# amorim-cleison/sign-language-nlp

Hardware: AMD Instinct MI355X
Metric: train seq/s (batch=50,len=48) (higher is better)
Workload: dtype bf16x3; 1 GPU; cfg2: Transformer train step E512 H8 N6 F512 batch 50 len 48 |src| 3000 |tgt| 202 dropout 0.1, fwd+CE+bwd+clip(0.5)+SGD(m=.9); launch=eager stream launches (auto: timed both in 9 untimed pre-warmup steps + warmup), per_gpu=independent fit (grid shard)

## Files before the change

include/slnlp.h:

```cpp
#ifndef SLNLP_H
#define SLNLP_H

#include <stdint.h>

#ifdef __cplusplus
extern "C" {
#endif

#define SLNLP_OK 0
#define SLNLP_ERR_INVALID_ARG 1
#define SLNLP_ERR_LAUNCH 2
#define SLNLP_ERR_UNSUPPORTED 3

#define SLNLP_ABI_VERSION 1

const char* slnlp_last_error(void);
int slnlp_abi_version(void);

typedef struct slnlp_gemm_args {
    const float* A; int64_t lda; int32_t a_kmajor;
    const float* B; int64_t ldb; int32_t b_kmajor;
    float* C; int64_t ldc;
    int32_t M, N, K;
    const float* bias;
// ... 466 lines not shown
    float dropout;
    int32_t precision;
} slnlp_tf_config;

int slnlp_tf_num_params(const slnlp_tf_config* cfg);
int slnlp_tf_param_info(const slnlp_tf_config* cfg, int i, char* name, int64_t shape[2], int* ndim,
                        int64_t* offset);
int64_t slnlp_tf_arena_floats(const slnlp_tf_config* cfg);
int64_t slnlp_tf_workspace_bytes(const slnlp_tf_config* cfg);

typedef struct slnlp_tf_buffers {
    float* params;
    float* grads;
    float* momentum;
    const float* pe;
    void* workspace;
    unsigned long long* rng;
    float* lr;
    float* scalars;
} slnlp_tf_buffers;

typedef struct slnlp_tf_plan slnlp_tf_plan;
int slnlp_tf_create(const slnlp_tf_config* cfg, const slnlp_tf_buffers* buf, slnlp_tf_plan** out);
void slnlp_tf_destroy(slnlp_tf_plan* plan);
int slnlp_tf_forward(slnlp_tf_plan* plan, const int64_t* X, const int64_t* y, int B, int train,
                     float* logp, void* stream);
int slnlp_tf_seed_dlogp(slnlp_tf_plan* plan, const float* dlogp, void* stream);
int slnlp_tf_backward(slnlp_tf_plan* plan, void* stream);
int slnlp_tf_optim(slnlp_tf_plan* plan, float momentum, float max_norm, void* stream);
int slnlp_tf_optim_adam(slnlp_tf_plan* plan, float* exp_avg_sq, float beta1, float beta2, float eps, float weight_decay,
                        float max_norm, void* stream);
int slnlp_tf_train_step(slnlp_tf_plan* plan, const int64_t* X, const int64_t* y, int B,
                        float momentum, float max_norm, float* logp, void* stream);
int slnlp_tf_graph_capture_train(slnlp_tf_plan* plan, const int64_t* X, const int64_t* y, int B,
                                 float momentum, float max_norm, float* logp, void* stream);
int slnlp_tf_graph_launch(slnlp_tf_plan* plan, int B, void* stream);
int slnlp_tf_tap(slnlp_tf_plan* plan, const char* name, float* out, int64_t max_floats,
                 int64_t* n_out, void* stream);
int slnlp_tf_params_changed(slnlp_tf_plan* plan);
int slnlp_tf_debug_layout(const slnlp_tf_config* cfg, char* out, int64_t out_bytes);

int slnlp_tf_set_destroy_sync(slnlp_tf_plan* plan, int on);

#define SLNLP_UPDATE_SGD 0
#define SLNLP_UPDATE_ADAM 1
#define SLNLP_UPDATE_ADAMW 2
int slnlp_tf_set_criterion(slnlp_tf_plan* plan, const float* class_weight, float label_smoothing, int reduction, void* stream);
int slnlp_tf_set_update(slnlp_tf_plan* plan, int kind, float dampening, float weight_decay, int nesterov);
int slnlp_tf_set_param_groups(slnlp_tf_plan* plan, int n_segments, const int64_t* seg_begin, const int32_t* seg_group,
                              int n_groups, const float* weight_decay, const float* lr_dev, void* stream);
int slnlp_tf_set_averaging(slnlp_tf_plan* plan, float* avg, float* count, int kind, float decay);
int slnlp_tf_set_dmem_batched(slnlp_tf_plan* plan, int on);
int slnlp_tf_set_dec_ln_fused(slnlp_tf_plan* plan, int on);

int slnlp_set_thread_stream_policy(int serialise);
int slnlp_set_stream_policy(int serialise);

int slnlp_set_backward_passes(int wgrad, int dgrad);
int slnlp_get_backward_passes(int* wgrad, int* dgrad);

typedef struct slnlp_timed_launch { int32_t blocks, njobs, geometry; float us; } slnlp_timed_launch;
int slnlp_launch_timer_start(int max_records);
int slnlp_launch_timer_stop(slnlp_timed_launch* out, int max_out);

typedef struct slnlp_tf_lockstep slnlp_tf_lockstep;
int64_t slnlp_tf_lockstep_workspace_bytes(const slnlp_tf_config* cfg, int K);
int slnlp_tf_lockstep_create(slnlp_tf_plan** plans, int K, void* workspace, int64_t workspace_bytes, void* stream,
                             slnlp_tf_lockstep** out);
void slnlp_tf_lockstep_destroy(slnlp_tf_lockstep* group);
int slnlp_tf_lockstep_set_data(slnlp_tf_lockstep* group, int slot, const int64_t* const* X, const int64_t* const* y,
                               int64_t rows, float* const* logp, float* const* loss, void* stream);
int slnlp_tf_lockstep_step(slnlp_tf_lockstep* group, int slot, int64_t row0, int B, int step_index, int train,
                           float momentum, float max_norm, void* stream);
int slnlp_tf_lockstep_epoch(slnlp_tf_lockstep* group, int slot, int batch, int train, float momentum, float max_norm,
                            void* stream);
int slnlp_tf_lockstep_num_launches(slnlp_tf_lockstep* group, int slot, int B, int train);
int slnlp_tf_lockstep_set_adam(slnlp_tf_lockstep* group, float* const* exp_avg_sq, float beta1, float beta2, float eps,
                               float weight_decay);
int slnlp_tf_lockstep_set_lr_table(slnlp_tf_lockstep* group, const float* const* table, int n_steps, void* stream);
int slnlp_tf_lockstep_set_order(slnlp_tf_lockstep* group, int slot, const int64_t* const* order, int64_t n_visit, void* stream);
int slnlp_tf_lockstep_set_averaging(slnlp_tf_lockstep* group, float* const* avg, float* const* count, int kind, float decay);
int slnlp_tf_lockstep_set_destroy_sync(slnlp_tf_lockstep* group, int on);


typedef struct slnlp_rnn_config {
    int32_t lstm;
    int32_t E, Hd, N;
    int32_t Vs, Vt, B, S;
    int32_t pad_src, pad_tgt, bos_idx;
    float dropout;
    int32_t precision;
} slnlp_rnn_config;
int slnlp_rnn_num_params(const slnlp_rnn_config* cfg);
int slnlp_rnn_param_info(const slnlp_rnn_config* cfg, int i, char* name, int64_t shape[2], int* ndim, int64_t* offset);
int64_t slnlp_rnn_arena_floats(const slnlp_rnn_config* cfg);
int64_t slnlp_rnn_workspace_bytes(const slnlp_rnn_config* cfg);
typedef struct slnlp_rnn_plan slnlp_rnn_plan;
int slnlp_rnn_create(const slnlp_rnn_config* cfg, const slnlp_tf_buffers* buf, slnlp_rnn_plan** out);
void slnlp_rnn_destroy(slnlp_rnn_plan* plan);
int slnlp_rnn_forward(slnlp_rnn_plan* plan, const int64_t* X, const int64_t* y, const int64_t* lengths, int B,
                      int train, float* logp, void* stream);
int slnlp_rnn_set_persistent(slnlp_rnn_plan* plan, int on);
int slnlp_rnn_set_fused_backward(slnlp_rnn_plan* plan, int on);
int slnlp_rnn_health(slnlp_rnn_plan* plan, int* status);
int slnlp_rnn_seed_dlogp(slnlp_rnn_plan* plan, const float* dlogp, void* stream);
int slnlp_rnn_backward(slnlp_rnn_plan* plan, void* stream);
// ... 41 lines not shown
```

sign-language-nlp_amd/csrc/elementwise.hip:

```cpp
#include "common.hpp"
#include "launch.hpp"
#include "layernorm_row.hpp"

namespace slnlp {

__device__ __forceinline__ void embed_fwd_body(const long* __restrict__ ids, long ld_ids, int B, int S,
                                                        int E, int V, const float* __restrict__ table,
                                                        const float* __restrict__ pe, float* __restrict__ out,
                                                        float scale, float drop_p, unsigned drop_thr, int drop_site,
                                                        const unsigned long long* __restrict__ rng, long nan_idx,
                                                        PlaneOut po, unsigned char* __restrict__ keep_mask) {
    const int e4 = E >> 2;
    const long total = (long)B * S * e4;
    const float ik = 1.f / (1.f - drop_p);
    for (long idx = blockIdx.x * 256L + threadIdx.x; idx < total; idx += (long)gridDim.x * 256) {
        const int m = (int)(idx / e4), c = (int)(idx % e4) * 4;
        const int s = m / B, b = m % B;
        const long id = ids[(long)b * ld_ids + s];
        float4 v = make_float4(0.f, 0.f, 0.f, 0.f);
        if (id >= 0 && id < V) v = *reinterpret_cast<const float4*>(table + id * E + c);
        const float4 p = pe ? *reinterpret_cast<const float4*>(pe + (long)s * E + c) : make_float4(0.f, 0.f, 0.f, 0.f);
        v.x = v.x * scale + p.x; v.y = v.y * scale + p.y; v.z = v.z * scale + p.z; v.w = v.w * scale + p.w;
        if (drop_p > 0.f) {
            const bool k0 = dropout_keep(rng, drop_site, m, c + 0, drop_thr), k1 = dropout_keep(rng, drop_site, m, c + 1, drop_thr);
// ... 37 lines not shown
    const int M = B * S, lane = threadIdx.x & 63;
    const int m = blockIdx.x, m0 = (m / EMB_CHUNK) * EMB_CHUNK, t = m - m0, mine = m0 + lane;
    int my_id = -1;
    if (mine < M) {
        const long v = ids[(long)(mine % B) * ld_ids + (mine / B)];
        my_id = (v < 0 || v >= V) ? -1 : (int)v;
    }
    const float ik = 1.f / (1.f - drop_p);
    const int id = __builtin_amdgcn_readlane(my_id, __builtin_amdgcn_readfirstlane(t));
    const unsigned long long mask = __ballot(my_id == id && id >= 0);
    const bool first = id >= 0 && (mask & ((1ull << t) - 1ull)) == 0ull;
    if (threadIdx.x == 0) pid[m] = first ? id : -1;
    if (!first) return;
    __shared__ __attribute__((aligned(16))) float red[4][256];
    const int wave = threadIdx.x >> 6;
    const unsigned long long wmask = mask & (0xFFFFull << (16 * wave));
    for (int c0 = 0; c0 < E; c0 += 256) {
        const int c = c0 + lane * 4;
        float4 acc = make_float4(0.f, 0.f, 0.f, 0.f);
        if (c < E) {
            unsigned long long bits = wmask;
            while (bits) {
                int k[4];
#pragma unroll
                for (int u = 0; u < 4; ++u) {
                    k[u] = bits ? __ffsll((long long)bits) - 1 : -1;
                    bits &= bits - 1;
                }
                float4 g[4];
#pragma unroll
                for (int u = 0; u < 4; ++u)
                    g[u] = k[u] >= 0 ? load_dx_row(dx, m0 + k[u], E, c, drop_p, ik, drop_thr, drop_site, rng, keep_mask)
                                     : make_float4(0.f, 0.f, 0.f, 0.f);
#pragma unroll
                for (int u = 0; u < 4; ++u) { acc.x += g[u].x; acc.y += g[u].y; acc.z += g[u].z; acc.w += g[u].w; }
            }
        }
        if (c0 > 0) __syncthreads();
        *reinterpret_cast<float4*>(&red[wave][lane * 4]) = acc;
        __syncthreads();
        if (wave == 0 && c < E) {
            float4 r = *reinterpret_cast<const float4*>(&red[0][lane * 4]);
#pragma unroll
            for (int w = 1; w < 4; ++w) {
                const float4 q = *reinterpret_cast<const float4*>(&red[w][lane * 4]);
                r.x += q.x; r.y += q.y; r.z += q.z; r.w += q.w;
            }
            *reinterpret_cast<float4*>(partial + (long)m * E + c) = r;
        }
    }
}
SLNLP_ZKERNEL(embed_bwd_chunk_kernel, 256, embed_bwd_chunk_body)

__device__ __forceinline__ void embed_bwd_combine_body(const int* __restrict__ pid, int M, int E,
                                                                const float* __restrict__ partial,
                                                                float* __restrict__ dtable, float scale) {
    __shared__ int list[1024];
    __shared__ int nlist;
    const int m = blockIdx.x, tid = threadIdx.x;
    const int id = pid[m];
    if (id < 0) return;
    int dup = 0;
    for (int mm = tid; mm < m; mm += 256) dup |= (pid[mm] == id);
    if (__syncthreads_or(dup)) return;
    if (tid == 0) nlist = 0;
    __syncthreads();
    for (int base = m; base < M; base += 256) {
        const int mm = base + tid;
        const bool hit = mm < M && pid[mm] == id;
        const unsigned long long bal = __ballot(hit);
        __shared__ unsigned long long match[4];
        __syncthreads();
        if ((tid & 63) == 0) match[tid >> 6] = bal;
        __syncthreads();
        if (tid == 0) {
            int n = nlist;
            for (int w = 0; w < 4; ++w) {
                unsigned long long bits = match[w];
                while (bits && n < 1024) {
                    list[n++] = base + w * 64 + __ffsll((long long)bits) - 1;
                    bits &= bits - 1;
                }
            }
            nlist = n;
        }
        __syncthreads();
    }
    const int n = nlist;
    __shared__ __attribute__((aligned(16))) float red[4][256];
    const int wave = tid >> 6, lane = tid & 63, per = (n + 3) / 4;
    const int i0 = wave * per, i1 = (i0 + per < n) ? i0 + per : n;
    for (int c0 = 0; c0 < E; c0 += 256) {
        const int c = c0 + lane * 4;
        float4 acc = make_float4(0.f, 0.f, 0.f, 0.f);
        if (c < E) {
            for (int i = i0; i < i1; i += 4) {
                float4 g[4];
#pragma unroll
                for (int u = 0; u < 4; ++u)
                    g[u] = (i + u < i1) ? *reinterpret_cast<const float4*>(partial + (long)list[i + u] * E + c)
                                        : make_float4(0.f, 0.f, 0.f, 0.f);
#pragma unroll
                for (int u = 0; u < 4; ++u) { acc.x += g[u].x; acc.y += g[u].y; acc.z += g[u].z; acc.w += g[u].w; }
            }
        }
        if (c0 > 0) __syncthreads();
        *reinterpret_cast<float4*>(&red[wave][lane * 4]) = acc;
        __syncthreads();
        if (wave == 0 && c < E) {
            float4 r = *reinterpret_cast<const float4*>(&red[0][lane * 4]);
#pragma unroll
            for (int w = 1; w < 4; ++w) {
                const float4 q = *reinterpret_cast<const float4*>(&red[w][lane * 4]);
                r.x += q.x; r.y += q.y; r.z += q.z; r.w += q.w;
            }
            r.x *= scale; r.y *= scale; r.z *= scale; r.w *= scale;
            *reinterpret_cast<float4*>(dtable + (long)id * E + c) = r;
        }
    }
}
SLNLP_ZKERNEL(embed_bwd_combine_kernel, 256, embed_bwd_combine_body)

__device__ __forceinline__ void embed_bwd_small_body(const long* __restrict__ ids, long ld_ids, int B, int S, int E, int V,
                                                     const float* __restrict__ dx, float* __restrict__ dtable, float scale,
                                                     float drop_p, unsigned drop_thr, int drop_site,
                                                     const unsigned long long* __restrict__ rng) {
    const int M = B * S, lane = threadIdx.x & 63, m = blockIdx.x;
    int my_id = -1;
    if (lane < M) {
        const long v = ids[(long)(lane % B) * ld_ids + (lane / B)];
        my_id = (v < 0 || v >= V) ? -1 : (int)v;
    }
    if (m < V && __ballot(my_id == m) == 0ull) {
        for (int c = threadIdx.x * 4; c < E; c += 1024) *reinterpret_cast<float4*>(dtable + (long)m * E + c) = make_float4(0.f, 0.f, 0.f, 0.f);
    }
    if (m >= M) return;
    const float ik = 1.f / (1.f - drop_p);
    const int id = __builtin_amdgcn_readlane(my_id, __builtin_amdgcn_readfirstlane(m));
    const unsigned long long mask = __ballot(my_id == id && id >= 0);
    const bool first = id >= 0 && (mask & ((1ull << m) - 1ull)) == 0ull;
    if (!first) return;
    __shared__ __attribute__((aligned(16))) float red[4][256];
    const int wave = threadIdx.x >> 6;
    const unsigned long long wmask = mask & (0xFFFFull << (16 * wave));
    for (int c0 = 0; c0 < E; c0 += 256) {
        const int c = c0 + lane * 4;
        float4 acc = make_float4(0.f, 0.f, 0.f, 0.f);
        if (c < E) {
            unsigned long long bits = wmask;
            while (bits) {
                int k[4];
#pragma unroll
                for (int u = 0; u < 4; ++u) {
                    k[u] = bits ? __ffsll((long long)bits) - 1 : -1;
                    bits &= bits - 1;
                }
// ... 256 lines not shown
    LnPartialEntry e = table ? table[blockIdx.y] : single;
    const float* __restrict__ dy = as_global(e.dy);
    const float* __restrict__ x = as_global(e.x);
    const float* __restrict__ stats = as_global(e.stats);
    float* __restrict__ partial = as_global(e.partial);
    const int rows = e.dec ? rows_dec : rows_enc, chunk = e.dec ? chunk_dec : chunk_enc;
    const int c = threadIdx.x * 4;
    if (c >= E || (int)blockIdx.x >= (e.dec ? nchunk_dec : nchunk_enc)) return;
    const int r0 = blockIdx.x * chunk;
    const int r1 = r0 + chunk < rows ? r0 + chunk : rows;
    float4 ag = make_float4(0.f, 0.f, 0.f, 0.f), ab = make_float4(0.f, 0.f, 0.f, 0.f);
    auto add = [&](const float4& dd, const float4& vv, float mean, float rstd) {
        ag.x += dd.x * ((vv.x - mean) * rstd); ag.y += dd.y * ((vv.y - mean) * rstd);
        ag.z += dd.z * ((vv.z - mean) * rstd); ag.w += dd.w * ((vv.w - mean) * rstd);
        ab.x += dd.x; ab.y += dd.y; ab.z += dd.z; ab.w += dd.w;
    };
    int r = r0;
    for (; r + 8 <= r1; r += 8) {
        float4 dd[8], vv[8];
        float2 ms[8];
#pragma unroll
        for (int i = 0; i < 8; ++i) {
            dd[i] = *reinterpret_cast<const float4*>(dy + (long)(r + i) * E + c);
            vv[i] = *reinterpret_cast<const float4*>(x + (long)(r + i) * E + c);
            ms[i] = *reinterpret_cast<const float2*>(stats + 2 * (r + i));
        }
#pragma unroll
        for (int i = 0; i < 8; ++i) add(dd[i], vv[i], ms[i].x, ms[i].y);
    }
    for (; r < r1; ++r)
        add(*reinterpret_cast<const float4*>(dy + (long)r * E + c), *reinterpret_cast<const float4*>(x + (long)r * E + c), stats[2 * r], stats[2 * r + 1]);
    *reinterpret_cast<float4*>(partial + ((long)blockIdx.x * 2 + 0) * E + c) = ag;
    *reinterpret_cast<float4*>(partial + ((long)blockIdx.x * 2 + 1) * E + c) = ab;
}
SLNLP_ZKERNEL(ln_param_partial_kernel, 256, ln_param_partial_body)

__device__ __forceinline__ void ln_param_reduce_body(const slnlp_ln_reduce_entry* __restrict__ table) {
    __shared__ float red[2][4][64];
    const slnlp_ln_reduce_entry e = table[blockIdx.x];
    const int col = threadIdx.x & 63, grp = threadIdx.x >> 6, c = blockIdx.y * 64 + col;
    float g = 0.f, b = 0.f;
    if (c < e.E) {
        int k = grp;
        for (; k + 28 < e.nblk; k += 32) {
            float pg[8], pb[8];
#pragma unroll
            for (int u = 0; u < 8; ++u) {
                pg[u] = e.partial[((long)(k + 4 * u) * 2 + 0) * e.E + c];
                pb[u] = e.partial[((long)(k + 4 * u) * 2 + 1) * e.E + c];
            }
#pragma unroll
            for (int u = 0; u < 8; ++u) { g += pg[u]; b += pb[u]; }
        }
        for (; k < e.nblk; k += 4) {
            g += e.partial[((long)k * 2 + 0) * e.E + c];
            b += e.partial[((long)k * 2 + 1) * e.E + c];
        }
    }
    red[0][grp][col] = g;
    red[1][grp][col] = b;
    __syncthreads();
    if (grp == 0 && c < e.E) {
        e.dgamma[c] = (red[0][0][col] + red[0][1][col]) + (red[0][2][col] + red[0][3][col]);
        e.dbeta[c] = (red[1][0][col] + red[1][1][col]) + (red[1][2][col] + red[1][3][col]);
    }
}
SLNLP_ZKERNEL(ln_param_reduce_kernel, 256, ln_param_reduce_body)

int layernorm_fwd(const float* x, const float* gamma, const float* beta, int rows, int E, float eps, float* y,
                  float* stats, hipStream_t st, PlaneOut po) {
    SLNLP_CHECK_ARG(x && gamma && beta && y, "layernorm_fwd: null pointer");
    SLNLP_CHECK_ARG(rows > 0 && E > 0 && E % 4 == 0 && E <= LN_MAXU * 256, "layernorm_fwd: need E %% 4 == 0 and E <= %d, got rows=%d E=%d", LN_MAXU * 256, rows, E);
    SLNLP_TRY(zlaunch(layernorm_fwd_kernel, dim3(ceil_div(rows, 4)), 256, 0, st, "layernorm_fwd",
                      x, gamma, beta, rows, E, eps, y, stats, po));
    return 0;
}

static int ln_bwd_group(int rows) { return rows >= 1024 ? 4 : 1; }

bool ln_bwd_fused(int full_rows) { return ln_bwd_group(full_rows) == 4; }
int ln_partial_chunk(int rows) {
    int c = 16;
    while (ceil_div(rows, c) > SLNLP_LN_MAX_PARTIALS) c *= 2;
    return c;
}
int ln_bwd_blocks(int rows) { return ceil_div(rows, ln_partial_chunk(rows)); }

int ln_param_partial(const LnPartialEntry* table_dev, const LnPartialEntry* single_host, int n, int E, int rows_enc, int rows_dec, int full_rows_enc,
                     int full_rows_dec, hipStream_t st) {
    SLNLP_CHECK_ARG(n > 0 && E > 0 && E % 4 == 0 && E <= LN_MAXU * 256, "ln_param_partial: bad args");
    LnPartialEntry single;
    memset(&single, 0, sizeof(single));
    if (single_host) single = *single_host;
    const int ce = ln_partial_chunk(full_rows_enc > 0 ? full_rows_enc : 1), cd = ln_partial_chunk(full_rows_dec > 0 ? full_rows_dec : 1);
    const int ne = full_rows_enc > 0 && !(table_dev && ln_bwd_fused(full_rows_enc)) ? ceil_div(full_rows_enc, ce) : 0;
    const int nd = full_rows_dec > 0 ? ceil_div(full_rows_dec, cd) : 0;
    const int nb = std::max(ne, nd);
    if (nb == 0) return 0;
    const int threads = (ceil_div(E, 4) + 63) / 64 * 64;
    return zlaunch(ln_param_partial_kernel, dim3(nb, n), threads, 0, st, "ln_param_partial", table_dev, single, E,
                   rows_enc, rows_dec, ce, cd, ne, nd);
}

int layernorm_bwd(const float* dy, const float* x, const float* gamma, const float* stats, int rows, int E,
                  const float* add_to_dx, float* dx, float* dx_drop, float drop_p, int drop_site,
                  const unsigned long long* rng, float* partial, int* nblk_out, int full_rows, hipStream_t st,
                  PlaneOut po_dx, PlaneOut po_drop) {
    SLNLP_CHECK_ARG(dy && x && gamma && stats && dx, "layernorm_bwd: null pointer");
    SLNLP_CHECK_ARG(rows > 0 && E > 0 && E % 4 == 0 && E <= LN_MAXU * 256, "layernorm_bwd: need E %% 4 == 0 and E <= %d, got %d", LN_MAXU * 256, E);
// ... 362 lines not shown
```

sign-language-nlp_amd/csrc/tf_plan.hip:

```cpp
#include <map>
#include <string>
#include <vector>

#include "common.hpp"
#include "launch.hpp"
#include "tf_plan.hpp"

using namespace slnlp;

extern "C" {

int slnlp_tf_num_params(const slnlp_tf_config* cfg) {
    if (check_cfg(cfg)) return -1;
    return (int)build_layout(*cfg).ents.size();
}

int slnlp_tf_param_info(const slnlp_tf_config* cfg, int i, char* name, int64_t shape[2], int* ndim, int64_t* offset) {
    SLNLP_TRY(check_cfg(cfg));
    return param_info(build_layout(*cfg).ents, i, "tf_param_info", name, shape, ndim, offset);
}

int64_t slnlp_tf_arena_floats(const slnlp_tf_config* cfg) {
    if (check_cfg(cfg)) return -1;
    return build_layout(*cfg).total;
}

int64_t slnlp_tf_workspace_bytes(const slnlp_tf_config* cfg) {
    if (check_cfg(cfg)) return -1;
    return (int64_t)carve(*cfg, nullptr).bytes;
}

void slnlp_tf_destroy(slnlp_tf_plan* plan) {
    if (plan) plan->destroy();
}

int slnlp_tf_create(const slnlp_tf_config* cfg, const slnlp_tf_buffers* buf, slnlp_tf_plan** out) {
    SLNLP_TRY(check_cfg(cfg));
    SLNLP_CHECK_ARG(buf && out, "tf_create: null argument");
    SLNLP_CHECK_ARG(buf->params && buf->grads && buf->momentum && buf->pe && buf->workspace && buf->rng && buf->lr &&
                        buf->scalars,
                    "tf_create: every buffer pointer is required");
    SLNLP_CHECK_ARG((((uintptr_t)buf->params | (uintptr_t)buf->grads | (uintptr_t)buf->momentum |
                      (uintptr_t)buf->workspace | (uintptr_t)buf->pe) & 255) == 0,
                    "tf_create: arenas / workspace / pe must be 256-byte aligned");
    slnlp_tf_plan* p = new slnlp_tf_plan();
    p->cfg = *cfg;
    p->buf = *buf;
    p->L = build_layout(*cfg);
    p->w = carve(*cfg, buf->workspace);
    p->arena = p->L.total; p->opt_partials = p->w.opt_partials;
    p->max_B = cfg->B; p->S = cfg->S; p->Vt = cfg->Vt; p->dropout = cfg->dropout;
    bool ok = attn_init() == 0 && gemm_planes_init() == 0;
    p->use_planes = (cfg->E % 64 == 0) && (cfg->F % 64 == 0);
    {
        const char* e = getenv("SLNLP_DEC_ROWS");
        p->use_rows = p->use_planes && cfg->E <= 1024 && cfg->F <= 1024 && !(e && atoi(e) == 0);
    }
    {
        const char* e = getenv("SLNLP_DEC_LN_FUSED");
        p->dec_ln_fused = !(e && atoi(e) == 0);
    }
    if (ok && cfg->precision == 8) {
        std::vector<QuantRow> rows;
        auto block = [&](long off, int nrows, int K) {
            p->qrow0[off] = (long)rows.size();
            for (int r = 0; r < nrows; ++r) rows.push_back(QuantRow{off + (long)r * K, K, 0});
        };
        const int E = cfg->E, F = cfg->F;
        for (int i = 0; i < cfg->N; ++i) {
            const EncP& q = p->L.enc[i];
            block(q.in_w, 3 * E, E); block(q.out_w, E, E); block(q.l1_w, F, E); block(q.l2_w, E, F);
        }
        ok = (long)rows.size() == p->w.n_qrows &&
             hipMemcpy(p->w.qrow_table, rows.data(), rows.size() * sizeof(QuantRow), hipMemcpyHostToDevice) == hipSuccess;
    }
    std::vector<slnlp_ln_reduce_entry> tab;
    std::vector<LnPartialEntry> ptab;
    const int nbE = p->nbE = ln_bwd_blocks(cfg->B * cfg->S), nbD = p->nbD = ln_bwd_blocks(cfg->B);
    auto ent = [&](float* part, long gw, long gb, int dec, const float* dy, const float* x, const float* stats) {
        slnlp_ln_reduce_entry e;
        e.partial = part; e.dgamma = p->G(gw); e.dbeta = p->G(gb); e.nblk = dec ? nbD : nbE; e.E = cfg->E;
        tab.push_back(e);
        LnPartialEntry q;
        q.dy = dy; q.x = x; q.stats = stats; q.partial = part; q.dec = dec; q.pad = 0;
        ptab.push_back(q);
    };
    {
        const Ws& w = p->w;
        const int N = cfg->N;
        for (int i = 0; i < N; ++i) {
            const EncA& a = w.enc[i];
            ent(a.lnp1, p->L.enc[i].n1_w, p->L.enc[i].n1_b, 0, a.gx1, a.y1, a.st1);
            ent(a.lnp2, p->L.enc[i].n2_w, p->L.enc[i].n2_b, 0, i + 1 < N ? w.enc[i + 1].gx0 : w.gxl, a.y2, a.st2);
        }
        ent(w.lnp_mem, p->L.encn_w, p->L.encn_b, 0, w.gmem, w.enc[N - 1].x2, w.st_mem);
        for (int i = 0; i < N; ++i) {
            const DecA& a = w.dec[i];
            ent(a.lnp1, p->L.dec[i].n1_w, p->L.dec[i].n1_b, 1, a.gt1, a.y1, a.st1);
            ent(a.lnp2, p->L.dec[i].n2_w, p->L.dec[i].n2_b, 1, a.gt2, a.y2, a.st2);
            ent(a.lnp3, p->L.dec[i].n3_w, p->L.dec[i].n3_b, 1, i + 1 < N ? w.dec[i + 1].gt0 : w.gtl, a.y3, a.st3);
        }
        ent(w.lnp_fin, p->L.decn_w, p->L.decn_b, 1, w.gfin, w.dec[N - 1].t3, w.st_fin);
    }
    std::vector<XmemDmemLayer> dtab;
    for (int i = 0; i < cfg->N; ++i) {
        const DecA& a = p->w.dec[i];
        XmemDmemLayer e;
        e.probs = a.xprobs; e.dsc = a.dsc; e.dmbar = a.dmbar; e.qk = a.qk; e.dcp = a.dcp;
        e.dbv = p->G(p->L.dec[i].cin_b) + 2 * cfg->E; e.drop_site = p->dec_site(i, 2); e.pad = 0;
        dtab.push_back(e);
    }
    ok = ok && hipMemcpy(p->w.dmem_tab, dtab.data(), dtab.size() * sizeof(dtab[0]), hipMemcpyHostToDevice) == hipSuccess;
    ok = ok && hipMemcpy(p->w.ln_table, tab.data(), tab.size() * sizeof(tab[0]), hipMemcpyHostToDevice) == hipSuccess &&
// ... 117 lines not shown
                            rng, nullptr, nullptr, 0, st));
    const float* dt = w.gtl;
    float* const gmem_l = pl->dmem_batched ? nullptr : w.gmem;
    const bool ur = pl->use_rows;
    for (int l = c.N - 1; l >= 0; --l) {
        const DecP& q = L.dec[l];
        const DecA& a = w.dec[l];
        const Mat t_in = l > 0 ? pl->rview(w.dec[l - 1].t3, w.dec[l - 1].t3p, E) : pl->rview(w.t0, w.t0p, E);
        SLNLP_TRY(pl->ln_bwd_dy(ur, dt, a.y3, q.n3_w, a.st3, B, a.gA3, a.gB3, a.d3p, p, pl->dec_site(l, 5), nullptr, 0, st));
        SLNLP_TRY(pl->linear_bwd(pl->rview(p > 0.f ? a.gB3 : a.gA3, a.d3p, E), q.l2_w, q.l2_b, pl->rview(a.h, a.hp, F), B, E, F, ur ? nullptr : a.gh,
                                 Epi().gated(a.h, ik).also(a.ghp), st));
        SLNLP_TRY(pl->linear_bwd(pl->rview(a.gh, a.ghp, F), q.l1_w, q.l1_b, pl->rview(a.t2, a.t2p, E), B, F, E, a.gt2, Epi().plus(a.gA3), st));
        SLNLP_TRY(pl->ln_bwd_dy(ur, a.gt2, a.y2, q.n2_w, a.st2, B, a.gA2, a.gB2, a.d2p, p, pl->dec_site(l, 3), nullptr, 0, st));
        SLNLP_TRY(pl->linear_bwd(pl->rview(p > 0.f ? a.gB2 : a.gA2, a.d2p, E), q.cout_w, q.cout_b, pl->rview(a.xctx, a.xctxp, E), B, E, E, a.gxctx, Epi(), st));
        {
            const float *Wk = pl->P(q.cin_w) + (long)E * E, *Wv = pl->P(q.cin_w) + 2L * E * E;
            const int pr = pl->prec3();
            const slnlp_gemm_args j1 = head_expand(a.gxctx, Wv, a.dmbar, B, H, dh, pr);
            SLNLP_TRY(gemm_group(&j1, 1, st));
            SLNLP_TRY(xmem_bwd(w.mem, pl->P(q.cin_b) + 2 * E, a.xprobs, a.psum, a.qk, a.dmbar, a.gxctx, B, S, H, dh, a.dsc, a.dqk, a.dcp,
                               pl->G(q.cin_b) + 2 * E, gmem_l, l == c.N - 1 ? 0 : 1, p, pl->dec_site(l, 2), rng, st));
            const slnlp_gemm_args jobs[3] = {head_reduce(a.dqk, Wk, a.gq, nullptr, ur ? &a.gqp : nullptr, B, H, dh, pr),
                                             head_wgrad(a.q, a.dqk, pl->G(q.cin_w) + (long)E * E, B, H, dh, pr),
                                             head_wgrad(a.gxctx, a.mbar, pl->G(q.cin_w) + 2L * E * E, B, H, dh, pr)};
            SLNLP_TRY(gemm_group(jobs, 3, st));
        }
        SLNLP_TRY(pl->linear_bwd(pl->rview(a.gq, a.gqp, E), q.cin_w, q.cin_b, pl->rview(a.t1, a.t1p, E), B, E, E, a.gt1, Epi().plus(a.gA2), st));
        SLNLP_TRY(pl->ln_bwd_dy(ur, a.gt1, a.y1, q.n1_w, a.st1, B, a.gA1, a.gB1, a.d1p, p, pl->dec_site(l, 1), nullptr, 0, st));
        SLNLP_TRY(pl->linear_bwd(pl->rview(p > 0.f ? a.gB1 : a.gA1, a.d1p, E), q.sout_w, q.sout_b, pl->rview(a.v, a.vp, E), B, E, E, ur ? nullptr : a.gv,
                                 Epi().dropped(p, pl->dec_site(l, 0), p > 0.f ? dh : 0).also(a.gvp), st));
        SLNLP_TRY(pl->linear_bwd(pl->rview(a.gv, a.gvp, E), q.sin_w + 2L * E * E, q.sin_b + 2 * E, t_in, B, E, E, a.gt0, Epi().plus(a.gA1), st));
        dt = a.gt0;
    }
    if (pl->dmem_batched) SLNLP_TRY(xmem_dmem_all(w.dmem_tab, c.N, B, S, H, dh, w.gmem, p, rng, st));
    SLNLP_TRY(embed_bwd(y, 1, B, 1, E, c.Vt, dt, pl->G(L.tgt_emb), sqrtf((float)E), -1, p, SITE_TGT_EMB, rng, w.emb_scratch_tgt, st));

    const int Mfull = c.B * c.S;
    const bool lnf = ln_bwd_fused(Mfull);
    SLNLP_TRY(layernorm_bwd(w.gmem, w.enc[c.N - 1].x2, pl->P(L.encn_w), w.st_mem, M, E, nullptr, w.gxl, nullptr, 0.f, 0,
                            rng, lnf ? w.lnp_mem : nullptr, nullptr, Mfull, st));
    const float* dx = w.gxl;
    for (int l = c.N - 1; l >= 0; --l) {
        const EncP& q = L.enc[l];
        const EncA& a = w.enc[l];
        SLNLP_TRY(pl->ln_bwd_dy(up, dx, a.y2, q.n2_w, a.st2, M, a.gA2, a.gB2, a.d2p, p, pl->enc_site(l, 3), lnf ? a.lnp2 : nullptr, Mfull, st));
        SLNLP_TRY(pl->enc_pair_launch(l, 0, B, st));
        SLNLP_TRY(pl->enc_pair_launch(l, 1, B, st));
        SLNLP_TRY(pl->ln_bwd_dy(up, a.gx1, a.y1, q.n1_w, a.st1, M, a.gA1, a.gB1, a.d1p, p, pl->enc_site(l, 1), lnf ? a.lnp1 : nullptr, Mfull, st));
        SLNLP_TRY(pl->enc_pair_launch(l, 2, B, st));
        SLNLP_TRY(attn_self_bwd(a.qkv, a.probs, a.gctx, B, S, H, dh, (up && S <= 64) ? nullptr : a.gqkv, p, pl->enc_site(l, 0), rng, st, pl->pout(a.gqkvp), w.attn_scratch));
        SLNLP_TRY(pl->enc_pair_launch(l, 3, B, st));
        dx = a.gx0;
    }
    if (up && !recording()) SLNLP_TRY(plane_batch_launch(pl->wbatch, w.wb_tab, w.wb_map, st));
    SLNLP_TRY(embed_bwd(X, S, B, S, E, c.Vs, dx, pl->G(L.src_emb), sqrtf((float)E), -1, p, SITE_SRC_EMB, rng, w.emb_scratch_src, st, w.emb_keep));
    SLNLP_TRY(ln_param_partial(w.ln_ptable, nullptr, 5 * c.N + 2, E, M, B, c.B * c.S, c.B, st));
    SLNLP_TRY(ln_param_reduce(w.ln_table, 5 * c.N + 2, E, st));
    return 0;
}

int slnlp_tf_optim(slnlp_tf_plan* pl, float momentum, float max_norm, void* stream) {
    SLNLP_CHECK_ARG(pl, "tf_optim: null plan");
    return pl->update_sgd(momentum, max_norm, (hipStream_t)stream);
}

int slnlp_tf_optim_adam(slnlp_tf_plan* pl, float* exp_avg_sq, float beta1, float beta2, float eps, float weight_decay,
                        float max_norm, void* stream) {
    SLNLP_CHECK_ARG(pl && exp_avg_sq, "tf_optim_adam: null argument");
    return pl->update_adam(exp_avg_sq, beta1, beta2, eps, weight_decay, max_norm, (hipStream_t)stream);
}

int slnlp_tf_set_destroy_sync(slnlp_tf_plan* pl, int on) {
    SLNLP_CHECK_ARG(pl, "tf_set_destroy_sync: null plan");
    pl->destroy_sync = on ? 1 : 0;
    return 0;
}

int slnlp_tf_set_dmem_batched(slnlp_tf_plan* pl, int on) {
    SLNLP_CHECK_ARG(pl, "tf_set_dmem_batched: null plan");
    if (pl->dmem_batched == (on != 0)) return 0;
    pl->dmem_batched = on != 0;
    ++pl->opts.gen;
    pl->drop_graphs();
    return 0;
}

int slnlp_tf_set_dec_ln_fused(slnlp_tf_plan* pl, int on) {
    SLNLP_CHECK_ARG(pl, "tf_set_dec_ln_fused: null plan");
    if (pl->dec_ln_fused == (on != 0)) return 0;
    pl->dec_ln_fused = on != 0;
    ++pl->opts.gen;
    pl->drop_graphs();
    return 0;
}

int slnlp_tf_set_criterion(slnlp_tf_plan* pl, const float* class_weight, float label_smoothing, int reduction, void* stream) {
    SLNLP_CHECK_ARG(pl, "tf_set_criterion: null plan");
    return pl->set_criterion(class_weight, label_smoothing, reduction, (hipStream_t)stream);
}

int slnlp_tf_set_update(slnlp_tf_plan* pl, int kind, float dampening, float weight_decay, int nesterov) {
    SLNLP_CHECK_ARG(pl, "tf_set_update: null plan");
    return pl->set_update(kind, dampening, weight_decay, nesterov);
}

int slnlp_tf_set_param_groups(slnlp_tf_plan* pl, int n_segments, const int64_t* seg_begin, const int32_t* seg_group, int n_groups,
                              const float* weight_decay, const float* lr_dev, void* stream) {
    SLNLP_CHECK_ARG(pl, "tf_set_param_groups: null plan");
    return pl->set_param_groups("tf_set_param_groups", n_segments, seg_begin, seg_group, n_groups, weight_decay, lr_dev, (hipStream_t)stream);
}

int slnlp_tf_set_averaging(slnlp_tf_plan* pl, float* avg, float* count, int kind, float decay) {
    SLNLP_CHECK_ARG(pl, "tf_set_averaging: null plan");
    return pl->set_averaging("tf_set_averaging", avg, count, kind, decay);
}

int slnlp_tf_params_changed(slnlp_tf_plan* pl) {
    SLNLP_CHECK_ARG(pl, "tf_params_changed: null plan");
    bump_params_generation(pl->buf.params);
    return 0;
}

int slnlp_tf_train_step(slnlp_tf_plan* pl, const int64_t* X, const int64_t* y, int B, float momentum, float max_norm,
                        float* logp, void* stream) {
    SLNLP_CHECK_ARG(pl, "tf_forward: `X` and `y` are required parameters");
    return pl->train_step(X, y, nullptr, B, momentum, max_norm, logp, (hipStream_t)stream);
}

int slnlp_tf_graph_capture_train(slnlp_tf_plan* pl, const int64_t* X, const int64_t* y, int B, float momentum,
                                 float max_norm, float* logp, void* stream) {
    SLNLP_CHECK_ARG(pl, "tf_graph_capture_train: needs a plan and a non-default stream");
    return pl->graph_capture_train("tf_graph_capture_train", X, y, nullptr, B, momentum, max_norm, logp, (hipStream_t)stream);
}

int slnlp_tf_graph_launch(slnlp_tf_plan* pl, int B, void* stream) {
// ... 92 lines not shown
```

sign-language-nlp_amd/csrc/tf_plan.hpp:

```cpp
#pragma once
#include <map>
#include <string>
#include <vector>

#include "common.hpp"
#include "gemm_jobs.hpp"
#include "launch.hpp"
#include "linear_jobs.hpp"
#include "plan_core.hpp"

namespace slnlp {

struct EncP { long in_w, in_b, out_w, out_b, l1_w, l1_b, l2_w, l2_b, n1_w, n1_b, n2_w, n2_b; };
struct DecP {
    long sin_w, sin_b, sout_w, sout_b, cin_w, cin_b, cout_w, cout_b, l1_w, l1_b, l2_w, l2_b;
    long n1_w, n1_b, n2_w, n2_b, n3_w, n3_b;
};
struct Layout {
    std::vector<ParamEnt> ents;
    long src_emb, tgt_emb, encn_w, encn_b, decn_w, decn_b, lin_w, lin_b, total;
    std::vector<EncP> enc;
    std::vector<DecP> dec;
};

// ... 271 lines not shown
    w.planes_begin = b.base + b.cur;
    w.x0p = pp(E, true);
    w.memp = pp(E, true);
    for (int i = 0; i < c.N; ++i) {
        EncA& a = w.enc[i];
        a.ctxp = pp(E, true); a.x1p = pp(E, true); a.hp = pp(F, true); a.x2p = pp(E, true);
        a.d2p = pp(E); a.ghp = pp(F); a.d1p = pp(E); a.gqkvp = pp(3 * E);
    }
    {
        const size_t Bp = (B + 63) / 64 * 64;
        auto ppd = [&](size_t cols) {
            PP q;
            q.hi = b.take<unsigned short>(Bp * cols);
            q.lo = b.take<unsigned short>(Bp * cols);
            return q;
        };
        w.t0p = ppd(E);
        w.tfinp = ppd(E);
        for (int i = 0; i < c.N; ++i) {
            DecA& a = w.dec[i];
            a.vp = ppd(E); a.t1p = ppd(E); a.xctxp = ppd(E); a.t2p = ppd(E); a.hp = ppd(F); a.t3p = ppd(E);
            a.d3p = ppd(E); a.ghp = ppd(F); a.d2p = ppd(E); a.gqp = ppd(E); a.d1p = ppd(E); a.gvp = ppd(E);
        }
    }
    {
        const size_t nx = ((E > F ? E : F) + 255) / 256 * 256, ny = ((3 * E > F ? 3 * E : F) + 255) / 256 * 256;
        w.gscr_bytes = 16384 + nx * ny * MAX_SPLITK * sizeof(float) + ny * MAX_SPLITK * sizeof(float);
        w.gscr_bytes = (w.gscr_bytes + 255) & ~(size_t)255;
        w.gscr[0] = b.take<char>(w.gscr_bytes);
        w.wb_scr_bytes = wb_jobs.empty() ? 0 : (plane_batch_scratch_bytes(wb_jobs.data(), wb_split.data(), (int)wb_jobs.size()) + 255) & ~(size_t)255;
        w.wb_scr = b.take<char>(w.wb_scr_bytes);
    }
    b.cur = (b.cur + 255) & ~(size_t)255;
    w.planes_end = b.base + b.cur;
    w.bytes = (b.cur + 255) & ~(size_t)255;
    return w;
}

}

using namespace slnlp;

enum { SITE_SRC_EMB = 1, SITE_TGT_EMB = 2, SITE_LAYER0 = 16, SITE_PER_LAYER = 8 };

struct slnlp_tf_plan : PlanCore {
    slnlp_tf_config cfg;
    Layout L;
    Ws w;
    const int64_t* last_X = nullptr;
    const int64_t* last_y = nullptr;
    int nbE = 0, nbD = 0;
    bool dmem_batched = true;
    bool dec_ln_fused = true;
    int prec3() const { return cfg.precision == 8 ? 3 : cfg.precision; }
    unsigned long long wq_gen = 0;
    std::map<long, long> qrow0;
    int ensure_wq(hipStream_t st) {
        if (cfg.precision != 8) return 0;
        unsigned long long g = params_generation(buf.params);
        if (g != 0 && g == wq_gen) return 0;
        SLNLP_TRY(quant_rows_fp8(buf.params, 0, (int)w.n_qrows, 0, w.wq, 0, w.wscale, w.qrow_table, st));
        if (g == 0) g = bump_params_generation(buf.params);
        wq_gen = g;
        return 0;
    }
    unsigned long long wplanes_gen = 0;
    int ensure_wplanes(hipStream_t st) {
        if (!use_planes) return 0;
        unsigned long long g = params_generation(buf.params);
        if (g != 0 && g == wplanes_gen) return 0;
        SLNLP_TRY(split_planes(buf.params, L.total, 1, (int)L.total, w.wp.hi, w.wp.lo, L.total, st));
        if (g == 0) g = bump_params_generation(buf.params);
        wplanes_gen = g;
        return 0;
    }
    long wplane_begin() const { return L.enc.empty() ? 0 : L.enc[0].in_w; }
    long wplane_end() const { return L.enc.empty() ? 0 : (use_rows && cfg.B <= ROWS_MAX_B ? L.encn_w : L.total); }
    static constexpr int ROWS_MAX_B = 64;
    bool rows_for(int B, int drop_head_dim) const { return B <= ROWS_MAX_B || drop_head_dim != 0; }
    void params_stepped() override {
        const unsigned long long g = bump_params_generation(buf.params);
        if (use_planes) wplanes_gen = g;
    }
    void before_capture() override { wplanes_gen = 0; }
    UpdateRanges update_ranges() const override {
        UpdateRanges r;
        if (use_planes) r.wp = w.wp.out();
        r.wp_begin = wplane_begin();
        r.wp_end = wplane_end();
        return r;
    }
    int prepare(int B, hipStream_t st) override {
        SLNLP_TRY(prepare_planes(B, st));
        SLNLP_TRY(ensure_wplanes(st));
        return ensure_wq(st);
    }
    bool same_shape(const PlanCore& other) const override {
        const slnlp_tf_config &c = cfg, &c0 = static_cast<const slnlp_tf_plan&>(other).cfg;
        return c.E == c0.E && c.H == c0.H && c.N == c0.N && c.F == c0.F && c.Vs == c0.Vs && c.Vt == c0.Vt && c.B == c0.B && c.S == c0.S &&
               c.precision == c0.precision && (c.dropout > 0.f) == (c0.dropout > 0.f);
    }
    int forward(const int64_t* X, const int64_t* y, const int64_t*, int B, int train, float* logp, hipStream_t st) override {
        return slnlp_tf_forward(this, X, y, B, train, logp, st);
    }
    int backward(hipStream_t st) override { return slnlp_tf_backward(this, st); }
    bool use_planes = false;
// ... 140 lines not shown
```

sign-language-nlp_amd/slnlp/_lib.py:

```python
import ctypes as C
import os

_HERE = os.path.dirname(os.path.abspath(__file__))
LIB_PATH = os.path.join(os.path.dirname(_HERE), "lib",
                        f"libslnlp_probe{os.environ['SLNLP_PROBE_LIB']}.so" if os.environ.get("SLNLP_PROBE_LIB") else "libslnlp.so")

i32, i64, f32, vp = C.c_int32, C.c_int64, C.c_float, C.c_void_p


class GemmArgs(C.Structure):
    _fields_ = [("A", vp), ("lda", i64), ("a_kmajor", i32),
                ("B", vp), ("ldb", i64), ("b_kmajor", i32),
                ("C", vp), ("ldc", i64),
                ("M", i32), ("N", i32), ("K", i32),
                ("bias", vp), ("relu", i32),
                ("gate", vp), ("ldg", i64), ("gate_scale", f32),
                ("drop_p", f32), ("drop_site", i32), ("rng", vp),
                ("resid", vp), ("ldr", i64),
                ("rowsum_a", vp), ("precision", i32), ("gate_mode", i32),
                ("A_hi", vp), ("A_lo", vp), ("lda_p", i64), ("B_hi", vp), ("B_lo", vp), ("ldb_p", i64),
                ("C_hi", vp), ("C_lo", vp), ("ldc_p", i64), ("drop_head_dim", i32),
                ("col_scale", vp), ("C_q8", vp),
                ("batch", i32), ("batch_stride_a", i64), ("batch_stride_b", i64), ("batch_stride_c", i64)]

# ... 173 lines not shown
    "slnlp_rnn_cell_bwd": (i32, [i32, C.POINTER(RnnCellBwdDir), i32, i32, i32, vp, i64, f32, i32, vp, vp]),
    "slnlp_rnn_step_bwd": (i32, [i32, C.POINTER(RnnStepBwdDir), i32, i32, i32, vp, i64, f32, i32, vp, i32, vp]),
    "slnlp_bahdanau_fwd": (i32, [vp, vp, vp, vp, vp, i64, i64, i32, i32, i32, vp, vp, vp]),
    "slnlp_bahdanau_bwd": (i32, [vp, vp, vp, vp, vp, vp, i32, i32, i32, vp, vp, vp, vp, vp, vp]),
    "slnlp_rnn_num_params": (i32, [C.POINTER(RnnConfig)]),
    "slnlp_rnn_param_info": (i32, [C.POINTER(RnnConfig), i32, C.c_char_p, C.POINTER(i64 * 2), C.POINTER(i32),
                                   C.POINTER(i64)]),
    "slnlp_rnn_arena_floats": (i64, [C.POINTER(RnnConfig)]),
    "slnlp_rnn_workspace_bytes": (i64, [C.POINTER(RnnConfig)]),
    "slnlp_rnn_create": (i32, [C.POINTER(RnnConfig), C.POINTER(TfBuffers), C.POINTER(vp)]),
    "slnlp_rnn_destroy": (None, [vp]),
    "slnlp_rnn_forward": (i32, [vp, vp, vp, vp, i32, i32, vp, vp]),
    "slnlp_rnn_seed_dlogp": (i32, [vp, vp, vp]),
    "slnlp_rnn_backward": (i32, [vp, vp]),
    "slnlp_rnn_optim": (i32, [vp, f32, f32, vp]),
    "slnlp_rnn_optim_adam": (i32, [vp, vp, f32, f32, f32, f32, f32, vp]),
    "slnlp_rnn_set_destroy_sync": (i32, [vp, i32]),
    "slnlp_rnn_set_criterion": (i32, [vp, vp, f32, i32, vp]),
    "slnlp_rnn_set_update": (i32, [vp, i32, f32, f32, i32]),
    "slnlp_rnn_set_param_groups": (i32, [vp, i32, vp, vp, i32, vp, vp, vp]),
    "slnlp_rnn_set_averaging": (i32, [vp, vp, vp, i32, f32]),
    "slnlp_rnn_train_step": (i32, [vp, vp, vp, vp, i32, f32, f32, vp, vp]),
    "slnlp_rnn_graph_capture_train": (i32, [vp, vp, vp, vp, i32, f32, f32, vp, vp]),
    "slnlp_rnn_graph_launch": (i32, [vp, i32, vp]),
    "slnlp_rnn_set_persistent": (i32, [vp, i32]),
    "slnlp_rnn_set_fused_backward": (i32, [vp, i32]),
    "slnlp_rnn_health": (i32, [vp, C.POINTER(i32)]),
    "slnlp_rnn_tap": (i32, [vp, C.c_char_p, vp, i64, C.POINTER(i64), vp]),
    "slnlp_tf_num_params": (i32, [C.POINTER(TfConfig)]),
    "slnlp_tf_param_info": (i32, [C.POINTER(TfConfig), i32, C.c_char_p, C.POINTER(i64 * 2), C.POINTER(i32),
                                  C.POINTER(i64)]),
    "slnlp_tf_arena_floats": (i64, [C.POINTER(TfConfig)]),
    "slnlp_tf_workspace_bytes": (i64, [C.POINTER(TfConfig)]),
    "slnlp_tf_create": (i32, [C.POINTER(TfConfig), C.POINTER(TfBuffers), C.POINTER(vp)]),
    "slnlp_tf_destroy": (None, [vp]),
    "slnlp_tf_forward": (i32, [vp, vp, vp, i32, i32, vp, vp]),
    "slnlp_tf_seed_dlogp": (i32, [vp, vp, vp]),
    "slnlp_tf_backward": (i32, [vp, vp]),
    "slnlp_tf_optim": (i32, [vp, f32, f32, vp]),
    "slnlp_tf_train_step": (i32, [vp, vp, vp, i32, f32, f32, vp, vp]),
    "slnlp_tf_graph_capture_train": (i32, [vp, vp, vp, i32, f32, f32, vp, vp]),
    "slnlp_tf_graph_launch": (i32, [vp, i32, vp]),
    "slnlp_tf_tap": (i32, [vp, C.c_char_p, vp, i64, C.POINTER(i64), vp]),
    "slnlp_tf_params_changed": (i32, [vp]),
    "slnlp_tf_optim_adam": (i32, [vp, vp, f32, f32, f32, f32, f32, vp]),
    "slnlp_tf_debug_layout": (i32, [vp, C.c_char_p, i64]),
    "slnlp_tf_set_destroy_sync": (i32, [vp, i32]),
    "slnlp_tf_set_criterion": (i32, [vp, vp, f32, i32, vp]),
    "slnlp_tf_set_update": (i32, [vp, i32, f32, f32, i32]),
    "slnlp_tf_set_param_groups": (i32, [vp, i32, vp, vp, i32, vp, vp, vp]),
    "slnlp_tf_set_averaging": (i32, [vp, vp, vp, i32, f32]),
    "slnlp_tf_set_dmem_batched": (i32, [vp, i32]),
    "slnlp_tf_set_dec_ln_fused": (i32, [vp, i32]),
    "slnlp_set_stream_policy": (i32, [i32]),
    "slnlp_set_thread_stream_policy": (i32, [i32]),
    "slnlp_set_backward_passes": (i32, [i32, i32]),
    "slnlp_get_backward_passes": (i32, [C.POINTER(i32), C.POINTER(i32)]),
    "slnlp_launch_timer_start": (i32, [i32]),
    "slnlp_launch_timer_stop": (i32, [C.POINTER(TimedLaunch), i32]),
    "slnlp_set_plane_tile": (i32, [i32]),
    "slnlp_plane_geo": (i32, [vp, vp, i32]),
    "slnlp_set_gemm_ks": (i32, [i32]),
    "slnlp_set_fp8_tile": (i32, [i32]),
    "slnlp_tf_lockstep_workspace_bytes": (i64, [vp, i32]),
    "slnlp_tf_lockstep_create": (i32, [vp, i32, vp, i64, vp, vp]),
    "slnlp_tf_lockstep_destroy": (None, [vp]),
    "slnlp_tf_lockstep_set_data": (i32, [vp, i32, vp, vp, i64, vp, vp, vp]),
    "slnlp_tf_lockstep_step": (i32, [vp, i32, i64, i32, i32, i32, C.c_float, C.c_float, vp]),
    "slnlp_tf_lockstep_epoch": (i32, [vp, i32, i32, i32, C.c_float, C.c_float, vp]),
    "slnlp_tf_lockstep_num_launches": (i32, [vp, i32, i32, i32]),
    "slnlp_tf_lockstep_set_adam": (i32, [vp, vp, f32, f32, f32, f32]),
    "slnlp_tf_lockstep_set_lr_table": (i32, [vp, vp, i32, vp]),
    "slnlp_tf_lockstep_set_order": (i32, [vp, i32, vp, i64, vp]),
    "slnlp_tf_lockstep_set_averaging": (i32, [vp, vp, vp, i32, f32]),
    "slnlp_tf_lockstep_set_destroy_sync": (i32, [vp, i32]),
    "slnlp_rnn_lockstep_workspace_bytes": (i64, [vp, i32]),
    "slnlp_rnn_lockstep_create": (i32, [vp, i32, vp, i64, vp, vp]),
    "slnlp_rnn_lockstep_destroy": (None, [vp]),
    "slnlp_rnn_lockstep_set_data": (i32, [vp, i32, vp, vp, vp, i64, vp, vp, vp]),
    "slnlp_rnn_lockstep_step": (i32, [vp, i32, i64, i32, i32, i32, C.c_float, C.c_float, vp]),
    "slnlp_rnn_lockstep_epoch": (i32, [vp, i32, i32, i32, C.c_float, C.c_float, vp]),
    "slnlp_rnn_lockstep_num_launches": (i32, [vp, i32, i32, i32]),
    "slnlp_rnn_lockstep_set_adam": (i32, [vp, vp, f32, f32, f32, f32]),
    "slnlp_rnn_lockstep_set_lr_table": (i32, [vp, vp, i32, vp]),
    "slnlp_rnn_lockstep_set_order": (i32, [vp, i32, vp, i64, vp]),
    "slnlp_rnn_lockstep_set_averaging": (i32, [vp, vp, vp, i32, f32]),
    "slnlp_rnn_lockstep_set_destroy_sync": (i32, [vp, i32]),
}

_lib = None


def load():
    global _lib
    if _lib is None:
        if not os.path.exists(LIB_PATH):
            raise RuntimeError(f"libslnlp.so not built at {LIB_PATH}: the HIP extension is the "
                               "only compute path (no CPU fallback)")
        lib = C.CDLL(LIB_PATH)
        for name, (res, args) in SIGNATURES.items():
            if os.environ.get("SLNLP_PROBE_LIB") and not hasattr(lib, name):
                continue
            fn = getattr(lib, name)
            fn.restype, fn.argtypes = res, args
        _lib = lib
    return _lib
# ... 75 lines not shown
```

Measured before the change: 21830 seq/s.

## Parallelise embed-grad combine list build, unroll LN reduce tail, reorder weight-plane batch

The embedding-gradient combine kernel now builds its duplicate-row list with per-wave ballot prefix counts across all threads, replacing the serial thread-0 scan. It also batches 8 ids per trip and sums 16 rows per inner iteration. The LN parameter reduce tail loop is unrolled into predicated loads. A new default-on option moves the weight-plane batch launch after the embedding and LN-parameter backward kernels. Together these aim to cut serialized latency in the backward tail, at the cost of more registers and shared-memory bookkeeping.

```diff
diff --git a/include/slnlp.h b/include/slnlp.h
--- a/include/slnlp.h
+++ b/include/slnlp.h
@@ -542,6 +542,7 @@
 int slnlp_tf_set_averaging(slnlp_tf_plan* plan, float* avg, float* count, int kind, float decay);
 int slnlp_tf_set_dmem_batched(slnlp_tf_plan* plan, int on);
 int slnlp_tf_set_dec_ln_fused(slnlp_tf_plan* plan, int on);
+int slnlp_tf_set_tail_first(slnlp_tf_plan* plan, int on);
 
 int slnlp_set_thread_stream_policy(int serialise);
 int slnlp_set_stream_policy(int serialise);
diff --git a/sign-language-nlp_amd/csrc/elementwise.hip b/sign-language-nlp_amd/csrc/elementwise.hip
--- a/sign-language-nlp_amd/csrc/elementwise.hip
+++ b/sign-language-nlp_amd/csrc/elementwise.hip
@@ -113,56 +113,73 @@
 }
 SLNLP_ZKERNEL(embed_bwd_chunk_kernel, 256, embed_bwd_chunk_body)
 
+constexpr int CMB_TRIPS = 8;
+constexpr int CMB_ROWS = 16;
 __device__ __forceinline__ void embed_bwd_combine_body(const int* __restrict__ pid, int M, int E,
                                                                 const float* __restrict__ partial,
                                                                 float* __restrict__ dtable, float scale) {
     __shared__ int list[1024];
-    __shared__ int nlist;
+    __shared__ int cnt[2][CMB_TRIPS][4];
     const int m = blockIdx.x, tid = threadIdx.x;
+    const int wave = __builtin_amdgcn_readfirstlane(tid >> 6), lane = tid & 63;
     const int id = pid[m];
     if (id < 0) return;
     int dup = 0;
-    for (int mm = tid; mm < m; mm += 256) dup |= (pid[mm] == id);
+    for (int base = 0; base < m; base += 256 * CMB_TRIPS) {
+        int v[CMB_TRIPS];
+#pragma unroll
+        for (int u = 0; u < CMB_TRIPS; ++u) {
+            const int mm = base + u * 256 + tid;
+            v[u] = mm < m ? pid[mm] : -1;
+        }
+#pragma unroll
+        for (int u = 0; u < CMB_TRIPS; ++u) dup |= (v[u] == id);
+    }
     if (__syncthreads_or(dup)) return;
-    if (tid == 0) nlist = 0;
+    int n = 0, pass = 0;
+    for (int base = m; base < M; base += 256 * CMB_TRIPS, pass ^= 1) {
+        unsigned long long bal[CMB_TRIPS];
+        int v[CMB_TRIPS];
+#pragma unroll
+        for (int u = 0; u < CMB_TRIPS; ++u) {
+            const int mm = base + u * 256 + tid;
+            v[u] = mm < M ? pid[mm] : -1;
+        }
+#pragma unroll
+        for (int u = 0; u < CMB_TRIPS; ++u) {
+            bal[u] = __ballot(v[u] == id);
+            if (lane == 0) cnt[pass][u][wave] = __popcll(bal[u]);
+        }
+        __syncthreads();
+#pragma unroll
+        for (int u = 0; u < CMB_TRIPS; ++u) {
+#pragma unroll
+            for (int w = 0; w < 4; ++w) {
+                if (w == wave && v[u] == id) {
+                    const int slot = n + __popcll(bal[u] & ((1ull << lane) - 1ull));
+                    if (slot < 1024) list[slot] = base + u * 256 + tid;
+                }
+                n += cnt[pass][u][w];
+            }
+        }
+    }
+    if (n > 1024) n = 1024;
     __syncthreads();
-    for (int base = m; base < M; base += 256) {
-        const int mm = base + tid;
-        const bool hit = mm < M && pid[mm] == id;
-        const unsigned long long bal = __ballot(hit);
-        __shared__ unsigned long long match[4];
-        __syncthreads();
-        if ((tid & 63) == 0) match[tid >> 6] = bal;
-        __syncthreads();
-        if (tid == 0) {
-            int n = nlist;
-            for (int w = 0; w < 4; ++w) {
-                unsigned long long bits = match[w];
-                while (bits && n < 1024) {
-                    list[n++] = base + w * 64 + __ffsll((long long)bits) - 1;
-                    bits &= bits - 1;
-                }
-            }
-            nlist = n;
-        }
-        __syncthreads();
-    }
-    const int n = nlist;
     __shared__ __attribute__((aligned(16))) float red[4][256];
-    const int wave = tid >> 6, lane = tid & 63, per = (n + 3) / 4;
+    const int per = (n + 3) / 4;
     const int i0 = wave * per, i1 = (i0 + per < n) ? i0 + per : n;
     for (int c0 = 0; c0 < E; c0 += 256) {
         const int c = c0 + lane * 4;
         float4 acc = make_float4(0.f, 0.f, 0.f, 0.f);
         if (c < E) {
-            for (int i = i0; i < i1; i += 4) {
-                float4 g[4];
-#pragma unroll
-                for (int u = 0; u < 4; ++u)
+            for (int i = i0; i < i1; i += CMB_ROWS) {
+                float4 g[CMB_ROWS];
+#pragma unroll
+                for (int u = 0; u < CMB_ROWS; ++u)
                     g[u] = (i + u < i1) ? *reinterpret_cast<const float4*>(partial + (long)list[i + u] * E + c)
                                         : make_float4(0.f, 0.f, 0.f, 0.f);
 #pragma unroll
-                for (int u = 0; u < 4; ++u) { acc.x += g[u].x; acc.y += g[u].y; acc.z += g[u].z; acc.w += g[u].w; }
+                for (int u = 0; u < CMB_ROWS; ++u) { acc.x += g[u].x; acc.y += g[u].y; acc.z += g[u].z; acc.w += g[u].w; }
             }
         }
         if (c0 > 0) __syncthreads();
@@ -525,9 +542,17 @@
 #pragma unroll
             for (int u = 0; u < 8; ++u) { g += pg[u]; b += pb[u]; }
         }
-        for (; k < e.nblk; k += 4) {
-            g += e.partial[((long)k * 2 + 0) * e.E + c];
-            b += e.partial[((long)k * 2 + 1) * e.E + c];
+        if (k < e.nblk) {
+            float pg[7], pb[7];
+#pragma unroll
+            for (int u = 0; u < 7; ++u) {
+                const bool in = k + 4 * u < e.nblk;
+                pg[u] = in ? e.partial[((long)(k + 4 * u) * 2 + 0) * e.E + c] : 0.f;
+                pb[u] = in ? e.partial[((long)(k + 4 * u) * 2 + 1) * e.E + c] : 0.f;
+            }
+#pragma unroll
+            for (int u = 0; u < 7; ++u)
+                if (k + 4 * u < e.nblk) { g += pg[u]; b += pb[u]; }
         }
     }
     red[0][grp][col] = g;
diff --git a/sign-language-nlp_amd/csrc/tf_plan.hip b/sign-language-nlp_amd/csrc/tf_plan.hip
--- a/sign-language-nlp_amd/csrc/tf_plan.hip
+++ b/sign-language-nlp_amd/csrc/tf_plan.hip
@@ -59,6 +59,10 @@
     {
         const char* e = getenv("SLNLP_DEC_LN_FUSED");
         p->dec_ln_fused = !(e && atoi(e) == 0);
+    }
+    {
+        const char* e = getenv("SLNLP_TAIL_FIRST");
+        p->tail_first = !(e && atoi(e) == 0);
     }
     if (ok && cfg->precision == 8) {
         std::vector<QuantRow> rows;
@@ -282,10 +286,12 @@
         SLNLP_TRY(pl->enc_pair_launch(l, 3, B, st));
         dx = a.gx0;
     }
-    if (up && !recording()) SLNLP_TRY(plane_batch_launch(pl->wbatch, w.wb_tab, w.wb_map, st));
+    const bool wb = up && !recording();
+    if (wb && !pl->tail_first) SLNLP_TRY(plane_batch_launch(pl->wbatch, w.wb_tab, w.wb_map, st));
     SLNLP_TRY(embed_bwd(X, S, B, S, E, c.Vs, dx, pl->G(L.src_emb), sqrtf((float)E), -1, p, SITE_SRC_EMB, rng, w.emb_scratch_src, st, w.emb_keep));
     SLNLP_TRY(ln_param_partial(w.ln_ptable, nullptr, 5 * c.N + 2, E, M, B, c.B * c.S, c.B, st));
     SLNLP_TRY(ln_param_reduce(w.ln_table, 5 * c.N + 2, E, st));
+    if (wb && pl->tail_first) SLNLP_TRY(plane_batch_launch(pl->wbatch, w.wb_tab, w.wb_map, st));
     return 0;
 }
 
@@ -311,6 +317,14 @@
     if (pl->dmem_batched == (on != 0)) return 0;
     pl->dmem_batched = on != 0;
     ++pl->opts.gen;
+    pl->drop_graphs();
+    return 0;
+}
+
+int slnlp_tf_set_tail_first(slnlp_tf_plan* pl, int on) {
+    SLNLP_CHECK_ARG(pl, "tf_set_tail_first: null plan");
+    if (pl->tail_first == (on != 0)) return 0;
+    pl->tail_first = on != 0;
     pl->drop_graphs();
     return 0;
 }
diff --git a/sign-language-nlp_amd/csrc/tf_plan.hpp b/sign-language-nlp_amd/csrc/tf_plan.hpp
--- a/sign-language-nlp_amd/csrc/tf_plan.hpp
+++ b/sign-language-nlp_amd/csrc/tf_plan.hpp
@@ -347,6 +347,7 @@
     int nbE = 0, nbD = 0;
     bool dmem_batched = true;
     bool dec_ln_fused = true;
+    bool tail_first = true;
     int prec3() const { return cfg.precision == 8 ? 3 : cfg.precision; }
     unsigned long long wq_gen = 0;
     std::map<long, long> qrow0;
diff --git a/sign-language-nlp_amd/slnlp/_lib.py b/sign-language-nlp_amd/slnlp/_lib.py
--- a/sign-language-nlp_amd/slnlp/_lib.py
+++ b/sign-language-nlp_amd/slnlp/_lib.py
@@ -249,6 +249,7 @@
     "slnlp_tf_set_averaging": (i32, [vp, vp, vp, i32, f32]),
     "slnlp_tf_set_dmem_batched": (i32, [vp, i32]),
     "slnlp_tf_set_dec_ln_fused": (i32, [vp, i32]),
+    "slnlp_tf_set_tail_first": (i32, [vp, i32]),
     "slnlp_set_stream_policy": (i32, [i32]),
     "slnlp_set_thread_stream_policy": (i32, [i32]),
     "slnlp_set_backward_passes": (i32, [i32, i32]),
```

Measured after the change: 21950 seq/s (median of 6 runs). About the same (+0.5%).
